# hellojialee/Improved-Body-Parts

Measured on NVIDIA H100. Metric: grouping images/sec @128x128 heatmaps, 30 persons/img, higher is better.
Workload: dtype f32 body-part maps, f32 keypoint maps; f64 coordinates/scores

## Files before the change

### improved_body_parts_b200/csrc/common.cuh

```cuda
#pragma once

#include <cuda_runtime.h>
#include <stdint.h>

#include <algorithm>

namespace spg {

#ifdef SPG_TRACE
constexpr int kTraceCtas = 64, kTraceSlots = 1024;
__device__ unsigned long long g_spg_trace[kTraceCtas * kTraceSlots];
__device__ __forceinline__ void trace_put(int slot, int dep, int mode) {
    if (blockIdx.x < kTraceCtas && (threadIdx.x & 31) == 0) {
        unsigned long long t;
        asm volatile("mov.u64 %0, %%clock64;" : "=l"(t) : "r"(dep) : "memory");
        unsigned long long *w = &g_spg_trace[blockIdx.x * kTraceSlots + slot];
        if (mode == 2) atomicCAS(w, 0ull, t);
        else if (mode == 3) atomicMax(w, t);
        else if (mode == 4) atomicAdd(w, (unsigned long long)(unsigned)dep);
        else *w = mode == 1 ? (unsigned long long)(unsigned)dep : t;
    }
}
#define SPG_TR(slot, dep) ::spg::trace_put((slot), (int)(dep), 0)
#define SPG_TRV(slot, v) ::spg::trace_put((slot), (int)(v), 1)
#define SPG_TR_FIRST(slot, dep) ::spg::trace_put((slot), (int)(dep), 2)
#define SPG_TR_LAST(slot, dep) ::spg::trace_put((slot), (int)(dep), 3)
#define SPG_TR_ADD(slot, v) ::spg::trace_put((slot), (int)(v), 4)
#else
#define SPG_TR(slot, dep) do {} while (0)
#define SPG_TRV(slot, v) do {} while (0)
#define SPG_TR_FIRST(slot, dep) do {} while (0)
#define SPG_TR_LAST(slot, dep) do {} while (0)
#define SPG_TR_ADD(slot, v) do {} while (0)
#endif

constexpr int kMaxParts = 32;
constexpr int kMaxLimbs = 64;
constexpr int kMaxCapPeaks = 128;
constexpr int kMaxCapRows = 128;
constexpr int kMaxRefineRadius = 4;
constexpr int kMaxOutJoints = 32;

constexpr uint32_t kStPeakOverflow = 1u << 0;
constexpr uint32_t kStCandOverflow = 1u << 1;
constexpr uint32_t kStRowOverflow = 1u << 2;
constexpr uint32_t kStSampleIndex = 1u << 3;
constexpr uint32_t kStAssert = 1u << 4;
constexpr uint32_t kStWireOverflow = 1u << 5;

struct Params {
    double thre1, thre2, connect_ration, len_rate, connection_tole, min_mean_score;
    int32_t mid_num, offset_radius, remove_recon, min_parts;
    int32_t crit1_strict, refresh_len_check;
};

struct Workspace {
    int K, L, J, capP, capC, capR, max_batch;
    int16_t limbs[kMaxLimbs * 2];
    int16_t out_from_part[kMaxOutJoints];
    double *peak_x, *peak_y;
    float *peak_score;
    uint32_t *peak_anchor;
    int32_t *peak_count;
    double *cand_prio, *cand_score;
    uint32_t *cand_ij;
    unsigned long long *cand_key;
    int32_t *cand_count;
    int32_t *surv_count;
    uint32_t *conn_ij;
    double *conn_score, *conn_norm;
    int32_t *conn_count;
    double *subset;
    int32_t *n_persons;
    double *people_xy;
    double *people_score;
    uint32_t *status;
    unsigned char *wire;
    long long wire_first;
    int wire_rows;
};

__device__ __forceinline__ uint32_t smem_u32(const void *p) { return (uint32_t)__cvta_generic_to_shared(p); }

__device__ __forceinline__ void mbar_init(uint64_t *bar, uint32_t count) {
    asm volatile("mbarrier.init.shared::cta.b64 [%0], %1;" ::"r"(smem_u32(bar)), "r"(count) : "memory");
}
__device__ __forceinline__ void fence_mbar_init() { asm volatile("fence.mbarrier_init.release.cluster;" ::: "memory"); }
__device__ __forceinline__ void fence_proxy_async() { asm volatile("fence.proxy.async.shared::cta;" ::: "memory"); }
__device__ __forceinline__ void mbar_expect_tx(uint64_t *bar, uint32_t bytes) {
    asm volatile("mbarrier.arrive.expect_tx.shared::cta.b64 _, [%0], %1;" ::"r"(smem_u32(bar)), "r"(bytes) : "memory");
}
__device__ __forceinline__ void bulk_g2s(void *dst_smem, const void *src_gmem, uint32_t bytes, uint64_t *bar) {
    asm volatile("cp.async.bulk.shared::cluster.global.mbarrier::complete_tx::bytes [%0], [%1], %2, [%3];" ::"r"(
                     smem_u32(dst_smem)),
                 "l"(src_gmem), "r"(bytes), "r"(smem_u32(bar))
                 : "memory");
}
__device__ __forceinline__ void mbar_arrive(uint64_t *bar) {
    asm volatile("mbarrier.arrive.shared::cta.b64 _, [%0];" ::"r"(smem_u32(bar)) : "memory");
}
__device__ __forceinline__ bool mbar_try_wait(uint64_t *bar, uint32_t parity) {
    uint32_t ok;
    asm volatile(
        "{\n"
        " .reg .pred p;\n"
        " mbarrier.try_wait.parity.shared::cta.b64 p, [%1], %2;\n"
        " selp.u32 %0, 1, 0, p;\n"
        "}\n"
        : "=r"(ok)
        : "r"(smem_u32(bar)), "r"(parity)
        : "memory");
    return ok != 0;
}
__device__ __forceinline__ void mbar_wait(uint64_t *bar, uint32_t parity) {
    while (!mbar_try_wait(bar, parity)) {
    }
}
__device__ __forceinline__ void mbar_wait_sleep(uint64_t *bar, uint32_t parity, uint32_t hint_ns = 20000u) {
    uint32_t ok = 0;
    while (!ok) {
        asm volatile(
            "{\n"
            " .reg .pred p;\n"
            " mbarrier.try_wait.parity.shared::cta.b64 p, [%1], %2, %3;\n"
            " selp.u32 %0, 1, 0, p;\n"
            "}\n"
            : "=r"(ok)
            : "r"(smem_u32(bar)), "r"(parity), "r"(hint_ns)
            : "memory");
    }
}

template <typename T>
__device__ __forceinline__ T pairwise_sum(const T *a, int n) {
    if (n < 8) {
        T res = (T)0;
        for (int i = 0; i < n; i++) res = res + a[i];
        return res;
    }
    T r[8];
#pragma unroll
    for (int k = 0; k < 8; k++) r[k] = a[k];
    int i = 8;
    for (; i < n - (n % 8); i += 8) {
#pragma unroll
        for (int k = 0; k < 8; k++) r[k] = r[k] + a[i + k];
    }
    T res = ((r[0] + r[1]) + (r[2] + r[3])) + ((r[4] + r[5]) + (r[6] + r[7]));
    for (; i < n; i++) res = res + a[i];
    return res;
}

}
```

### improved_body_parts_b200/csrc/limb_score_persist.cuh

```cuda
#pragma once

#include "limb_score.cuh"

namespace spg {

constexpr int kPersistThreads = 1024;
constexpr int kPersistSlots = 3;
constexpr int kMetaSlots = 5;
constexpr int kWorkerWarps = kPersistThreads / 32 - 1;
constexpr int kPersistMaxCapP = 64;
constexpr int kScreenTailBypass = 4;
constexpr int kPersistListCap = 1024;

constexpr int kTrItemWords = 16, kTrItems = 64;
#define SPG_TR_ITEM(kind, j, f, dep) do { if ((j) < kTrItems) kind(kTrItemWords * (j) + (f), dep); } while (0)

struct PersistHdr {
    int nA, nB, npairs, n, k, special;
    uint32_t magic;
    int pad;
};

struct alignas(16) PeakSlot {
    double ax[kPersistMaxCapP], ay[kPersistMaxCapP], bx[kPersistMaxCapP], by[kPersistMaxCapP];
    float as[kPersistMaxCapP], bs[kPersistMaxCapP];
    float2 fa[kPersistMaxCapP], fb[kPersistMaxCapP];
    unsigned char ain[kPersistMaxCapP], bin[kPersistMaxCapP];
};

struct alignas(16) MetaSlot {
    PeakSlot peaks;
    uint16_t list[kPersistListCap];
    PersistHdr hdr;
    int nsurv, ncand, bnext;
    uint32_t flags;
};

constexpr size_t kPersistPlaneOffset = (screen_tables_bytes() + kMetaSlots * sizeof(MetaSlot) + 127) & ~(size_t)127;
inline size_t persist_smem_bytes(size_t plane_bytes, int ) {
    const size_t plane = (plane_bytes + 127) & ~(size_t)127;
    return kPersistPlaneOffset + kPersistSlots * plane + 128;
}

constexpr uint32_t kScreenBias = 0x4B400000u >> 6;

struct ScreenCtx {
    const PeakSlot *ps;
    uint32_t base;
    const ScreenTab *tab;
    const float *ts;
    int W, mid_num, nB;
    uint32_t magic;
    float thre2;
};

__device__ __forceinline__ void screen_pair(const ScreenCtx &c, int pc, bool valid, int &fails, int &qn, int &maxfail) {
    const int i = c.nB > 1 ? (int)__umulhi((uint32_t)pc, c.magic) : pc;
    const int jj = pc - i * c.nB;
    const float2 fa = c.ps->fa[i], fb = c.ps->fb[jj];
    const float dx64 = fb.x - fa.x, dy64 = fb.y - fa.y;
    const float n2 = (dx64 * dx64 + dy64 * dy64) * (1.0f / 4096.0f);
    float rs;
    asm("rsqrt.approx.ftz.f32 %0, %1;" : "=f"(rs) : "f"(n2));
    const float qf = n2 * rs + 1.0f;
    const float r = rintf(qf);
    const bool longp = qf >= (float)c.mid_num + 0.51f;
    int m = longp ? c.mid_num : min((int)r, c.mid_num);
    if (!longp && !(fabsf(qf - r) < 0.49f)) m = 0;
    if (!(n2 > 1e-6f) || !valid || fminf(fa.x, fb.x) < 0.0f) m = 0;
    m = max(m, 0);
    const ScreenTab tb = c.tab[m];
    qn = tb.qn;
    maxfail = tb.maxfail;
    const float sx64 = dx64 * tb.inv, sy64 = dy64 * tb.inv;
    const float ax64o = fa.x + 33.0f, ay64o = fa.y + 33.0f;
    const float *ts = c.ts + m * kScreenSamples;
    const int qmax = __reduce_max_sync(0xffffffffu, qn);
    const uint32_t base = c.base;
    fails = 0;
    auto sample = [&](int q2) {
        const float tf = ts[q2];
        const uint32_t xb = __float_as_uint(__fadd_rn(__fmaf_rn(tf, sx64, ax64o), 12582912.0f));
        const uint32_t yb = __float_as_uint(__fadd_rn(__fmaf_rn(tf, sy64, ay64o), 12582912.0f));
        float v;
        asm("ld.shared.f32 %0, [%1];" : "=f"(v) : "r"(base + 4u * ((yb >> 6) * (uint32_t)c.W + (xb >> 6))));
        fails += (int)(min(xb & 63u, yb & 63u) > 2u) & (int)!(v > c.thre2);
    };
    if (qmax == kScreenSamples) {
#pragma unroll
        for (int q2 = 0; q2 < kScreenSamples; q2++) sample(q2);
    } else {
#pragma unroll
        for (int q2 = 0; q2 < kScreenSamples; q2++) {
            if (q2 >= qmax) break;
            sample(q2);
        }
    }
    maxfail += qmax - qn;
}

template <typename TA>
__global__ void __launch_bounds__(kPersistThreads, 1) limb_score_persist_kernel(ScoreArgs a, int n_items) {
    extern __shared__ __align__(128) unsigned char smem_raw[];
    __shared__ uint64_t bar_full[kPersistSlots], bar_screened[kMetaSlots], bar_mfree[kMetaSlots];
    __shared__ uint32_t s_bias_bytes;

    using T = float;
    const Workspace &ws = a.ws;
    const int tid = threadIdx.x, lane = tid & 31, warp = tid >> 5;
    const int H = a.H, W = a.W, capP = ws.capP, L = ws.L;
    const size_t plane_bytes = (size_t)H * W * sizeof(T);
    const size_t plane_stride = (plane_bytes + 127) & ~(size_t)127;
    double *s_rcp = reinterpret_cast<double *>(smem_raw);
    ScreenTab *s_tab = reinterpret_cast<ScreenTab *>(s_rcp + (kScreenMaxMid + 1));
    float *s_ts = reinterpret_cast<float *>(s_tab + (kScreenMaxMid + 1));
    MetaSlot *s_meta = reinterpret_cast<MetaSlot *>(smem_raw + screen_tables_bytes());
    unsigned char *s_planes = smem_raw + kPersistPlaneOffset;
    const int nE = min(max(a.exact_warps, 1), kWorkerWarps - 1), nS = kWorkerWarps - nE;

    if (tid == 0) {
        for (int s = 0; s < kPersistSlots; s++) {
            mbar_init(&bar_full[s], 2);
        }
        for (int e = 0; e < kMetaSlots; e++) {
            mbar_init(&bar_screened[e], nS);
            mbar_init(&bar_mfree[e], nE);
            s_meta[e].nsurv = 0; s_meta[e].ncand = 0; s_meta[e].bnext = 0; s_meta[e].flags = 0;
        }
        s_bias_bytes = 4u * kScreenBias * (uint32_t)(W + 1);
        fence_mbar_init();
    }
    if (tid >= 32 && tid < 32 + kScreenMaxMid + 1) build_screen_row(a, tid - 32, s_rcp, s_tab, s_ts, true);
    __syncthreads();

    const int G = gridDim.x;
    const int nj = ((int)blockIdx.x < n_items) ? (n_items - 1 - (int)blockIdx.x) / G + 1 : 0;
    const bool screen = a.screen && a.mid_num <= kScreenMaxMid && H <= kScreenMaxDim && W <= kScreenMaxDim;
    const T thre2 = sizeof(TA) == 8 ? f32_not_above(a.thre2) : (T)a.thre2;
    const TA thre2_exact = (TA)a.thre2;
    auto plane_of = [&](int n_local, int k) {
        return reinterpret_cast<const T *>(a.paf) + (int64_t)n_local * a.img_stride + (int64_t)k * a.chan_stride;
    };

    if (warp == 0) {
        constexpr int kMaxE = kPersistMaxCapP / 32;
        double r_xa[kMaxE], r_ya[kMaxE], r_xb[kMaxE], r_yb[kMaxE];
        float r_sa[kMaxE], r_sb[kMaxE];
        int r_cntA = 0, r_cntB = 0;
        auto fetch = [&](int j) {
            const int item = (int)blockIdx.x + j * G;
            const int n_local = item / L, k = item - n_local * L;
            const int n = a.image_base + n_local;
            const int pa = ws.limbs[2 * k], pb = ws.limbs[2 * k + 1];
            r_cntA = ws.peak_count[(size_t)n * ws.K + pa];
            r_cntB = ws.peak_count[(size_t)n * ws.K + pb];
            const size_t baseA = ((size_t)n * ws.K + pa) * capP, baseB = ((size_t)n * ws.K + pb) * capP;
#pragma unroll
            for (int u = 0; u < kMaxE; u++) {
                const int e = lane + 32 * u;
                if (e < capP) {
                    r_xa[u] = ws.peak_x[baseA + e]; r_ya[u] = ws.peak_y[baseA + e];
                    r_xb[u] = ws.peak_x[baseB + e]; r_yb[u] = ws.peak_y[baseB + e];
                    r_sa[u] = ws.peak_score[baseA + e]; r_sb[u] = ws.peak_score[baseB + e];
                }
            }
        };
        auto close_item = [&](int jp) {
            if (lane == 0) {
                MetaSlot &ms = s_meta[jp % kMetaSlots];
                SPG_TR_ITEM(SPG_TR, jp, 8, ms.nsurv);
                SPG_TR_ITEM(SPG_TRV, jp, 9, ms.nsurv);
                SPG_TR_ITEM(SPG_TRV, jp, 10, ms.ncand);
                publish_limb(ws, ms.hdr.n, (size_t)ms.hdr.n * L + ms.hdr.k, ms.hdr.special ? -1 : ms.ncand, ms.nsurv, ms.flags);
                ms.nsurv = 0; ms.ncand = 0; ms.bnext = 0; ms.flags = 0;
            }
            __syncwarp();
        };
        if (nj > 0) fetch(0);
        for (int j = 0; j < nj; j++) {
            const int s = j % kPersistSlots, e = j % kMetaSlots;
            SPG_TR_ITEM(SPG_TR, j, 0, j);
            if (j >= kPersistSlots) {
                const int jp = j - kPersistSlots;
                mbar_wait_sleep(&bar_screened[jp % kMetaSlots], (jp / kMetaSlots) & 1);
            }
            const int item = (int)blockIdx.x + j * G;
            const int n_local = item / L, k = item - n_local * L;
            const int n = a.image_base + n_local;
            if (lane == 0) {
                const unsigned char *gplane = reinterpret_cast<const unsigned char *>(plane_of(n_local, k));
                unsigned char *dst = s_planes + s * plane_stride;
                mbar_expect_tx(&bar_full[s], (uint32_t)plane_bytes);
                for (size_t off = 0; off < plane_bytes; off += kBulkChunkBytes) {
                    const uint32_t bytes = (uint32_t)min((size_t)kBulkChunkBytes, plane_bytes - off);
                    bulk_g2s(dst + off, gplane + off, bytes, &bar_full[s]);
                }
            }
            SPG_TR_ITEM(SPG_TR, j, 1, j);
            if (j >= kMetaSlots) {
                SPG_TR_ITEM(SPG_TR, j, 2, j);
                mbar_wait_sleep(&bar_mfree[e], ((j / kMetaSlots) - 1) & 1);
                SPG_TR_ITEM(SPG_TR, j, 3, j);
                close_item(j - kMetaSlots);
            }
            MetaSlot &ms = s_meta[e];
            PeakSlot &ps = ms.peaks;
#pragma unroll
            for (int u = 0; u < kMaxE; u++) {
                const int q = lane + 32 * u;
                if (q < capP) {
                    const double xa = r_xa[u], ya = r_ya[u], xb = r_xb[u], yb = r_yb[u];
                    ps.ax[q] = xa; ps.ay[q] = ya; ps.bx[q] = xb; ps.by[q] = yb;
                    ps.as[q] = r_sa[u]; ps.bs[q] = r_sb[u];
                    const bool ain = inside_map(xa, ya, H, W), bin = inside_map(xb, yb, H, W);
                    ps.fa[q] = ain ? make_float2((float)(xa * 64.0), (float)(ya * 64.0)) : make_float2(-1.0f, 0.0f);
                    ps.fb[q] = bin ? make_float2((float)(xb * 64.0), (float)(yb * 64.0)) : make_float2(-1.0f, 0.0f);
                    ps.ain[q] = ain;
                    ps.bin[q] = bin;
                }
            }
            const int nA = min(r_cntA, capP), nB = min(r_cntB, capP);
            const bool special = nA == 0 || nB == 0;
            if (lane == 0) {
                PersistHdr h;
                h.nA = nA; h.nB = nB; h.npairs = special ? 0 : nA * nB; h.n = n; h.k = k; h.special = special;
                h.magic = nB > 1 ? 0xffffffffu / (uint32_t)nB + 1u : 0u;
                h.pad = 0;
                ms.hdr = h;
            }
            __syncwarp();
            SPG_TR_ITEM(SPG_TR, j, 4, j);
            if (lane == 0) mbar_arrive(&bar_full[s]);
            if (j + 1 < nj) fetch(j + 1);
        }
        for (int jp = max(0, nj - kMetaSlots); jp < nj; jp++) {
            mbar_wait_sleep(&bar_mfree[jp % kMetaSlots], (jp / kMetaSlots) & 1);
            close_item(jp);
        }
    } else {
        auto exact_one = [&](MetaSlot &ms, const T *plane, int p) {
            const PersistHdr &h = ms.hdr;
            const PeakSlot &ps = ms.peaks;
            const int nB = h.nB;
            const int i = nB > 1 ? (int)__umulhi((uint32_t)p, h.magic) : p;
            const int jj = p - i * nB;
            PairGeom g{ps.ax, ps.ay, ps.bx, ps.by, ps.as, ps.bs, s_rcp};
            double score, prio;
            bool bad = false;
            const bool ok = score_pair_exact<T, 10, TA>(plane, H, W, a, g, i, jj, ps.ain[i] && ps.bin[jj], thre2_exact, score, prio, bad);
            if (bad) atomicOr(&ms.flags, kStSampleIndex);
            if (ok) {
                const size_t out_base = ((size_t)h.n * L + h.k) * ws.capC;
                const int pos = atomicAdd(&ms.ncand, 1);
                if (pos < ws.capC) store_candidate<TA>(ws, out_base, pos, i, jj, score, prio);
            }
        };

        if (warp <= nS) {
            int c0 = warp - 1;
            for (int j = 0; j < nj; j++) {
                const int s = j % kPersistSlots, e = j % kMetaSlots;
                mbar_wait_sleep(&bar_full[s], (j / kPersistSlots) & 1);
                SPG_TR_ITEM(SPG_TR_FIRST, j, 5, j);
                MetaSlot &ms = s_meta[e];
                const int npairs = ms.hdr.npairs;
                if (c0 * 32 < npairs) {
                    const T *plane = reinterpret_cast<const T *>(s_planes + s * plane_stride);
                    const ScreenCtx sc{&ms.peaks, smem_u32(plane) - *(volatile uint32_t *)&s_bias_bytes, s_tab, s_ts, W, a.mid_num,
                                       ms.hdr.nB, ms.hdr.magic, thre2};
                    for (int c = c0; c * 32 < npairs; c += nS) {
                        const int p = c * 32 + lane;
                        bool keep = p < npairs;
                        if (screen && npairs - c * 32 > kScreenTailBypass) {
                            int fails, qn, maxfail;
                            screen_pair(sc, min(p, npairs - 1), keep, fails, qn, maxfail);
                            if (qn > 0) keep = fails <= maxfail;
                        }
                        const uint32_t km = __ballot_sync(0xffffffffu, keep);
                        if (km) {
                            int at = 0;
                            if (lane == 0) at = atomicAdd(&ms.nsurv, __popc(km));
                            at = __shfl_sync(0xffffffffu, at, 0);
                            if (keep) {
                                const int at_me = at + __popc(km & ((1u << lane) - 1u));
                                if (at_me < kPersistListCap) ms.list[at_me] = (uint16_t)p;
                                else exact_one(ms, plane, p);
                            }
                        }
                    }
                }
                __syncwarp();
                SPG_TR_ITEM(SPG_TR_FIRST, j, 6, j);
                SPG_TR_ITEM(SPG_TR_LAST, j, 7, j);
                if (lane == 0) mbar_arrive(&bar_screened[e]);
                if (++c0 == nS) c0 = 0;
            }
        } else {
            for (int j = 0; j < nj; j++) {
                const int e = j % kMetaSlots;
                mbar_wait_sleep(&bar_screened[e], (j / kMetaSlots) & 1);
                MetaSlot &ms = s_meta[e];
                const int ns = min(ms.nsurv, kPersistListCap);
                if (ns > 0) {
                    const T *gplane = plane_of(ms.hdr.n - a.image_base, ms.hdr.k);
                    for (;;) {
                        if (*(volatile int *)&ms.bnext * 32 >= ns) break;
                        int c = 0;
                        if (lane == 0) c = atomicAdd(&ms.bnext, 1);
                        c = __shfl_sync(0xffffffffu, c, 0);
                        if (c * 32 >= ns) break;
                        const int t = c * 32 + lane;
                        if (t < ns) exact_one(ms, gplane, ms.list[t]);
                        __syncwarp();
                    }
                }
                __syncwarp();
                SPG_TR_ITEM(SPG_TR_LAST, j, 11, j);
                if (lane == 0) mbar_arrive(&bar_mfree[e]);
            }
        }
    }
}

}
```

### improved_body_parts_b200/csrc/spgroup.cu

```cuda
#include "../../include/spgroup.h"

#include <cuda_runtime.h>

#include <algorithm>
#include <cmath>
#include <cstdarg>
#include <cstdio>
#include <cstdlib>
#include <cstring>
#include <new>
#include <string>
#include <vector>

#include "assemble.cuh"
#include "common.cuh"
#include "limb_match.cuh"
#include "limb_score.cuh"
#include "limb_score_persist.cuh"
#include "match_assemble.cuh"
#include "nms_peaks.cuh"
#include "nms_peaks_persist.cuh"
#include "nms_peaks_banded.cuh"
#include "postnet.cuh"
#include "prenet.cuh"

using namespace spg;

static_assert(sizeof(spg_params) == sizeof(spg::Params), "spg_params layout");

static thread_local std::string g_create_error;

enum : int { kStageNms, kStageScore, kStageMatch, kStageAssemble, kStagePostnet, kStagePrenet, kStageCount };

struct Scratch {
    void *p = nullptr;
    size_t bytes = 0;
};

struct spg_handle {
    spg_config cfg{};
    int device = 0;
    int sm_count = 0;
    size_t smem_optin = 0;
    Workspace ws{};
    std::vector<void *> allocs;
    Scratch in_heat, in_paf;
    unsigned int *done_counter = nullptr;
    unsigned long long *armed_flag = nullptr;
    unsigned long long armed_value = 0;
    Scratch heat_acc;
    Scratch pre_grid;
    cudaStream_t streams[2] = {nullptr, nullptr};
    int64_t launches = 0;
    const char *stage_kernel[kStageCount] = {"", "", "", "", "", ""};
    int persist = 1;
    int screen = 1;
    int exact_warps = 14;
    int ma_warps = kMAMatchWarps;
    int fuse_ma = 1;
    int cand_dtype = SPG_F32;
    int stage = 0;
    std::string err;
};

namespace {

int fail(spg_handle *h, int code, const char *fmt, ...) {
    char buf[512];
    va_list ap;
    va_start(ap, fmt);
    vsnprintf(buf, sizeof buf, fmt, ap);
    va_end(ap);
    if (h) h->err = buf; else g_create_error = buf;
    return code;
}

#define SPG_CUDA(h, call)                                                                              \
    do {                                                                                               \
        cudaError_t e_ = (call);                                                                       \
        if (e_ != cudaSuccess) return fail((h), SPG_E_CUDA, "%s failed: %s", #call, cudaGetErrorString(e_)); \
    } while (0)

template <typename T>
int dalloc(spg_handle *h, T **p, size_t count) {
    void *q = nullptr;
    SPG_CUDA(h, cudaMalloc(&q, std::max<size_t>(count, 1) * sizeof(T)));
    h->allocs.push_back(q);
    *p = static_cast<T *>(q);
    return SPG_OK;
}

struct DeviceGuard {
    int prev = -1;
    explicit DeviceGuard(int dev) {
        cudaGetDevice(&prev);
        if (prev != dev) cudaSetDevice(dev);
    }
    ~DeviceGuard() {
        int cur = -1;
        cudaGetDevice(&cur);
        if (prev >= 0 && cur != prev) cudaSetDevice(prev);
    }
};

int grow(spg_handle *h, Scratch &s, size_t bytes) {
    if (s.bytes >= bytes) return SPG_OK;
    if (s.p) cudaFree(s.p);
    s.p = nullptr;
    s.bytes = 0;
    SPG_CUDA(h, cudaMalloc(&s.p, bytes));
    s.bytes = bytes;
    return SPG_OK;
}

template <typename... P, typename... A>
int launch(spg_handle *h, int stage, const char *name, void (*kern)(P...), dim3 grid, int block, size_t smem, cudaStream_t st,
           const A &...args) {
    if (smem > 0) SPG_CUDA(h, cudaFuncSetAttribute(kern, cudaFuncAttributeMaxDynamicSharedMemorySize, (int)smem));
    kern<<<grid, block, smem, st>>>(args...);
    h->stage_kernel[stage] = name;
    h->launches++;
    SPG_CUDA(h, cudaGetLastError());
    return SPG_OK;
}

int check_batch(spg_handle *h, int n) {
    if (n < 0 || n > h->cfg.max_batch) return fail(h, SPG_E_INVALID, "n_images %d outside [0, max_batch=%d]", n, h->cfg.max_batch);
    return SPG_OK;
}

int check_dims(spg_handle *h, int n, int H, int W) {
    int rc;
    if ((rc = check_batch(h, n))) return rc;
    if (H < 2 || W < 2 || H > h->cfg.max_h || W > h->cfg.max_w || H > 32767 || W > 32767)
        return fail(h, SPG_E_INVALID, "map %dx%d outside [2, %dx%d]", H, W, h->cfg.max_h, h->cfg.max_w);
    return SPG_OK;
}

int check_params(spg_handle *h, const spg_params *p) {
    if (!p) return fail(h, SPG_E_INVALID, "params is NULL");
    if (p->offset_radius < 0 || p->offset_radius > kMaxRefineRadius)
        return fail(h, SPG_E_INVALID, "offset_radius %d outside [0, %d]", p->offset_radius, kMaxRefineRadius);
    if (p->mid_num < 1) return fail(h, SPG_E_INVALID, "mid_num must be >= 1");
    return SPG_OK;
}

int check_dtype(spg_handle *h, int dtype) {
    if (dtype != SPG_F32 && dtype != SPG_F64 && dtype != SPG_F32_AS_F64)
        return fail(h, SPG_E_INVALID, "paf_dtype must be SPG_F32, SPG_F64 or SPG_F32_AS_F64");
    return SPG_OK;
}

struct ScoreKernels {
    size_t esz;
    void (*item[2])(ScoreArgs);
    const char *item_name[2];
    void (*ragged[2])(ScoreArgs, ScoreRagged);
    const char *ragged_name[2];
    void (*persist)(ScoreArgs, int);
    const char *persist_name;
};

static_assert(SPG_F32 == 0 && SPG_F64 == 1 && SPG_F32_AS_F64 == 2, "kScoreKernels is indexed by the dtype");
const ScoreKernels kScoreKernels[3] = {
    {4, {limb_score_kernel<float, false>, limb_score_kernel<float, true>},
     {"limb_score_kernel<float,false>", "limb_score_kernel<float,true>"},
     {limb_score_ragged_kernel<float, false>, limb_score_ragged_kernel<float, true>},
     {"limb_score_ragged_kernel<float,false>", "limb_score_ragged_kernel<float,true>"},
     limb_score_persist_kernel<float>, "limb_score_persist_kernel<float>"},
    {8, {limb_score_kernel<double, false>, limb_score_kernel<double, true>},
     {"limb_score_kernel<double,false>", "limb_score_kernel<double,true>"},
     {limb_score_ragged_kernel<double, false>, limb_score_ragged_kernel<double, true>},
     {"limb_score_ragged_kernel<double,false>", "limb_score_ragged_kernel<double,true>"},
     nullptr, ""},
    {4, {limb_score_kernel<float, false, double>, limb_score_kernel<float, true, double>},
     {"limb_score_kernel<float,false,double>", "limb_score_kernel<float,true,double>"},
     {limb_score_ragged_kernel<float, false, double>, limb_score_ragged_kernel<float, true, double>},
     {"limb_score_ragged_kernel<float,false,double>", "limb_score_ragged_kernel<float,true,double>"},
     limb_score_persist_kernel<double>, "limb_score_persist_kernel<double>"},
};

void (*const kNmsPersistKernels[])(NmsArgs, int) = {nms_peaks_persist_kernel<0>, nms_peaks_persist_kernel<1>, nms_peaks_persist_kernel<2>,
                                                    nms_peaks_persist_kernel<3>, nms_peaks_persist_kernel<4>};
static_assert(kMaxRefineRadius == 4, "one nms_peaks_persist_kernel instantiation per radius");

struct NmsPlan {
    enum { kPersist, kBanded, kBands } kind;
    int band_rows, use_bulk;
    size_t smem;
    NmsBanding bg;
};

int plan_nms(spg_handle *h, const float *heat, int64_t img_stride, int64_t chan_stride, int H, int W, bool persistent, int image,
             NmsPlan *pl) {
    const int capP = h->ws.capP;
    *pl = NmsPlan{};
    pl->use_bulk = (W % 4 == 0) && (img_stride % 4 == 0) && (chan_stride % 4 == 0) && ((reinterpret_cast<uintptr_t>(heat) & 15) == 0);
    const bool persist = persistent && h->persist && pl->use_bulk;
    if (persist && nms_persist_smem_bytes(H, W, capP) <= h->smem_optin && (size_t)H * W / 4 < 65536 &&
        (size_t)H * W * sizeof(float) < (1u << 20) &&
        ((size_t)H * W / 4 + kNmsPScanners - 1) / kNmsPScanners <= (size_t)32 * kNmsPMaxIter) {
        pl->kind = NmsPlan::kPersist;
        pl->smem = nms_persist_smem_bytes(H, W, capP);
        return SPG_OK;
    }
    if (persist) pl->bg = nms_banding(H, W, capP, h->smem_optin - 1024);
    if (pl->bg.slots >= kNmsBTeams) {
        pl->kind = NmsPlan::kBanded;
        pl->band_rows = pl->bg.band_rows;
        pl->smem = pl->bg.smem;
        return SPG_OK;
    }
    pl->kind = NmsPlan::kBands;
    pl->band_rows = std::max(4, std::min(H, 4096 / W));
    pl->smem = nms_smem_bytes(pl->band_rows, H, W, capP);
    if (pl->smem <= h->smem_optin) return SPG_OK;
    if (image < 0)
        return fail(h, SPG_E_INVALID, "map width %d needs %zu B of shared memory per band (limit %zu)", W, pl->smem, h->smem_optin);
    return fail(h, SPG_E_INVALID, "image %d: map width %d needs %zu B of shared memory per band (limit %zu)", image, W, pl->smem,
                h->smem_optin);
}

struct ScorePlan {
    enum { kSampled, kStaged, kPersist } kind;
    size_t smem;
};

ScorePlan plan_score(const spg_handle *h, const ScoreKernels &k, const void *paf, int64_t img_stride, int64_t chan_stride, int H,
                     int W, bool persistent) {
    const int capP = h->ws.capP;
    const size_t plane_bytes = (size_t)H * W * k.esz;
    const bool aligned = (plane_bytes % 16 == 0) && ((img_stride * k.esz) % 16 == 0) && ((chan_stride * k.esz) % 16 == 0) &&
                         ((reinterpret_cast<uintptr_t>(paf) & 15) == 0) && plane_bytes < (1u << 20);
    if (persistent && h->persist && k.persist && aligned && capP <= kPersistMaxCapP && persist_smem_bytes(plane_bytes, capP) <= h->smem_optin)
        return {ScorePlan::kPersist, persist_smem_bytes(plane_bytes, capP)};
    const size_t staged = score_smem_bytes(plane_bytes, capP);
    if (aligned && staged <= h->smem_optin) return {ScorePlan::kStaged, staged};
    return {ScorePlan::kSampled, score_smem_bytes(0, capP)};
}

NmsArgs nms_args(const spg_handle *h, const spg_params *p) {
    NmsArgs a{};
    a.radius = p->offset_radius;
    a.thr = (float)p->thre1;
    a.ws = h->ws;
    return a;
}

ScoreArgs score_args(const spg_handle *h, const spg_params *p) {
    ScoreArgs a{};
    a.mid_num = p->mid_num;
    a.thre2 = p->thre2;
    a.connect_ration = p->connect_ration;
    a.screen = h->screen;
    a.crit1_strict = p->crit1_strict != 0;
    a.exact_warps = h->exact_warps;
    a.ws = h->ws;
    return a;
}

AssembleArgs assemble_args(const spg_handle *h, int base, int n, const spg_params *p) {
    AssembleArgs a{};
    a.n_images = n;
    a.image_base = base;
    a.len_rate = p->len_rate;
    a.connection_tole = p->connection_tole;
    a.min_mean_score = p->min_mean_score;
    a.remove_recon = p->remove_recon;
    a.min_parts = p->min_parts;
    a.refresh_len_check = p->refresh_len_check != 0;
    a.wire_flag = h->armed_flag; a.wire_flag_value = h->armed_value; a.done_counter = h->done_counter;
    a.ws = h->ws;
    a.ws.wire_first += base;
    return a;
}

int launch_nms(spg_handle *h, const float *heat, int64_t img_stride, int64_t chan_stride, int base, int n, int H, int W,
               const spg_params *p, cudaStream_t st) {
    if (n == 0) return SPG_OK;
    NmsPlan pl;
    int rc;
    if ((rc = plan_nms(h, heat, img_stride, chan_stride, H, W, true, -1, &pl))) return rc;
    NmsArgs a = nms_args(h, p);
    a.heat = heat;
    a.img_stride = img_stride;
    a.chan_stride = chan_stride;
    a.H = H;
    a.W = W;
    a.band_rows = pl.band_rows;
    a.use_bulk = pl.use_bulk;
    a.image_base = base;
    const int items = n * h->ws.K;
    switch (pl.kind) {
        case NmsPlan::kPersist:
            return launch(h, kStageNms, "nms_peaks_persist_kernel", kNmsPersistKernels[a.radius], std::min(items, h->sm_count),
                          kNmsPThreads, pl.smem, st, a, items);
        case NmsPlan::kBanded:
            return launch(h, kStageNms, "nms_peaks_banded_kernel", nms_peaks_banded_kernel, std::min(items, h->sm_count), kNmsPThreads,
                          pl.smem, st, a, items, pl.bg.slots, pl.bg.n_bands);
        default:
            return launch(h, kStageNms, "nms_peaks_kernel", nms_peaks_kernel, items, kNmsThreads, pl.smem, st, a);
    }
}

int launch_score(spg_handle *h, const void *paf, int dtype, int64_t img_stride, int64_t chan_stride, int base, int n, int H,
                 int W, double extent, const spg_params *p, cudaStream_t st) {
    if (n == 0) return SPG_OK;
    const ScoreKernels &k = kScoreKernels[dtype];
    ScoreArgs a = score_args(h, p);
    a.paf = paf;
    a.img_stride = img_stride;
    a.chan_stride = chan_stride;
    a.H = H;
    a.W = W;
    a.image_base = base;
    a.image_extent = extent;
    h->cand_dtype = dtype;
    const ScorePlan pl = plan_score(h, k, paf, img_stride, chan_stride, H, W, true);
    const int grid = n * h->ws.L;
    if (pl.kind == ScorePlan::kPersist)
        return launch(h, kStageScore, k.persist_name, k.persist, std::min(grid, h->sm_count), kPersistThreads, pl.smem, st, a, grid);
    return launch(h, kStageScore, k.item_name[pl.kind], k.item[pl.kind], grid, kScoreThreads, pl.smem, st, a);
}

template <typename Args, typename Ragged, typename Image>
int launch_ragged(spg_handle *h, int stage, const char *name, void (*kern)(Args, Ragged), int per_image, int block, size_t smem,
                  cudaStream_t st, const Args &a, const std::vector<Image> &imgs) {
    constexpr size_t cap = sizeof(Ragged::img) / sizeof(Image);
    for (size_t i0 = 0; i0 < imgs.size(); i0 += cap) {
        const size_t cnt = std::min(cap, imgs.size() - i0);
        Ragged r{};
        std::copy(imgs.begin() + i0, imgs.begin() + i0 + cnt, r.img);
        int rc;
        if ((rc = launch(h, stage, name, kern, (int)cnt * per_image, block, smem, st, a, r))) return rc;
    }
    return SPG_OK;
}

int launch_match(spg_handle *h, int base, int n, cudaStream_t st) {
    if (n == 0) return SPG_OK;
    MatchArgs a{};
    a.n_images = n;
    a.image_base = base;
    a.keys_valid = h->cand_dtype == SPG_F32;
    a.ws = h->ws;
    const int warps = n * h->ws.L;
    const int blocks = (warps * 32 + kMatchThreads - 1) / kMatchThreads;
    return launch(h, kStageMatch, "limb_match_kernel", limb_match_kernel, blocks, kMatchThreads, 0, st, a);
}

int launch_assemble(spg_handle *h, int base, int n, const spg_params *p, cudaStream_t st) {
    if (n == 0) return SPG_OK;
    AssembleArgs a = assemble_args(h, base, n, p);
    h->armed_flag = nullptr;
    a.use_bulk = ((size_t)h->ws.L * h->ws.capP * sizeof(uint32_t)) % 16 == 0;
    const size_t smem = assemble_smem_bytes(h->ws.K, h->ws.capP, h->ws.capR) + assemble_conn_bytes(h->ws.L, h->ws.capP);
    if (smem > h->smem_optin) return fail(h, SPG_E_INVALID, "capacities need %zu B of shared memory in assemble (limit %zu)", smem, h->smem_optin);
    return launch(h, kStageAssemble, "assemble_kernel", assemble_kernel, n, kAssembleThreads, smem, st, a);
}

int launch_match_assemble(spg_handle *h, int base, int n, const spg_params *p, cudaStream_t st) {
    if (n == 0) return SPG_OK;
    AssembleArgs a = assemble_args(h, base, n, p);
    a.use_bulk = ((size_t)h->ws.K * h->ws.capP * sizeof(float)) % 16 == 0;
    const size_t smem = match_assemble_smem_bytes(h->ws.K, h->ws.L, h->ws.capP, h->ws.capR, h->ma_warps);
    if (smem > h->smem_optin) {
        int rc;
        if ((rc = launch_match(h, base, n, st))) return rc;
        return launch_assemble(h, base, n, p, st);
    }
    h->armed_flag = nullptr;
    h->stage_kernel[kStageAssemble] = "";
    return launch(h, kStageMatch, "match_assemble_kernel", match_assemble_kernel, n, 32 * (1 + h->ma_warps), smem, st, a,
                  h->cand_dtype == SPG_F32);
}

int launch_people(spg_handle *h, int base, int n, const spg_params *p, cudaStream_t st) {
    if (h->fuse_ma) return launch_match_assemble(h, base, n, p, st);
    int rc;
    if ((rc = launch_match(h, base, n, st))) return rc;
    return launch_assemble(h, base, n, p, st);
}

int run_all(spg_handle *h, const float *heat, int64_t his, int64_t hcs, const void *paf, int dtype, int64_t pis, int64_t pcs,
            int base, int n, int H, int W, double extent, const spg_params *p, cudaStream_t st) {
    int rc;
    SPG_CUDA(h, cudaMemsetAsync(h->ws.status + base, 0, sizeof(uint32_t) * (size_t)n, st));
    if ((rc = launch_nms(h, heat, his, hcs, base, n, H, W, p, st))) return rc;
    if ((rc = launch_score(h, paf, dtype, pis, pcs, base, n, H, W, extent, p, st))) return rc;
    return launch_people(h, base, n, p, st);
}

__global__ void wire_signal_kernel(unsigned long long *word, unsigned long long value) {
    __threadfence_system();
    asm volatile("st.release.sys.global.u64 [%0], %1;" ::"l"(word), "l"(value) : "memory");
}

struct WireWords {
    unsigned long long *p[32];
    int n;
};
__global__ void wire_signal_many_kernel(WireWords w, unsigned long long value) {
    __threadfence_system();
    if ((int)threadIdx.x < w.n) asm volatile("st.release.sys.global.u64 [%0], %1;" ::"l"(w.p[threadIdx.x]), "l"(value) : "memory");
}

__global__ void wire_wait_kernel(const unsigned long long *word, unsigned long long value) {
    unsigned long long v;
    do {
        asm volatile("ld.acquire.sys.global.u64 %0, [%1];" : "=l"(v) : "l"(word) : "memory");
        if (v < value) __nanosleep(500);
    } while (v < value);
}

}

extern "C" {

#ifdef SPG_TRACE
int spg_trace_read(unsigned long long *out, size_t n_words, int clear) {
    const size_t n = std::min(n_words, (size_t)spg::kTraceCtas * spg::kTraceSlots);
    if (cudaMemcpyFromSymbol(out, spg::g_spg_trace, n * sizeof(unsigned long long)) != cudaSuccess) return -1;
    if (clear) {
        void *p = nullptr;
        if (cudaGetSymbolAddress(&p, spg::g_spg_trace) != cudaSuccess) return -1;
        if (cudaMemset(p, 0, sizeof(spg::g_spg_trace)) != cudaSuccess) return -1;
    }
    return 0;
}
#endif

int spg_abi_version(void) { return SPG_ABI_VERSION; }

const char *spg_last_error(const spg_handle *h) { return h ? h->err.c_str() : g_create_error.c_str(); }

int spg_create(const spg_config *cfg, spg_handle **out) {
    if (!cfg || !out) return fail(nullptr, SPG_E_INVALID, "cfg/out is NULL");
    *out = nullptr;
    if (cfg->abi_version != SPG_ABI_VERSION) return fail(nullptr, SPG_E_INVALID, "ABI version %d != %d", cfg->abi_version, SPG_ABI_VERSION);
    if (cfg->n_parts < 1 || cfg->n_parts > kMaxParts || cfg->n_limbs < 1 || cfg->n_limbs > kMaxLimbs || !cfg->limbs)
        return fail(nullptr, SPG_E_INVALID, "n_parts in [1,%d], n_limbs in [1,%d], limbs non-NULL required", kMaxParts, kMaxLimbs);
    if (cfg->n_out_joints < 0 || cfg->n_out_joints > kMaxOutJoints || (cfg->n_out_joints && !cfg->out_from_part))
        return fail(nullptr, SPG_E_INVALID, "n_out_joints in [0,%d]", kMaxOutJoints);
    if (cfg->max_peaks_per_part < 1 || cfg->max_peaks_per_part > kMaxCapPeaks)
        return fail(nullptr, SPG_E_INVALID, "max_peaks_per_part in [1,%d]", kMaxCapPeaks);
    if (cfg->max_person_rows < 1 || cfg->max_person_rows > kMaxCapRows)
        return fail(nullptr, SPG_E_INVALID, "max_person_rows in [1,%d]", kMaxCapRows);
    if (cfg->max_cands_per_limb < 1 || cfg->max_batch < 1 || cfg->max_h < 2 || cfg->max_w < 2)
        return fail(nullptr, SPG_E_INVALID, "max_cands_per_limb, max_batch >= 1 and max_h, max_w >= 2 required");
    for (int k = 0; k < cfg->n_limbs * 2; k++)
        if (cfg->limbs[k] < 0 || cfg->limbs[k] >= cfg->n_parts) return fail(nullptr, SPG_E_INVALID, "limb table entry %d out of range", k);
    for (int g = 0; g < cfg->n_out_joints; g++)
        if (cfg->out_from_part[g] < 0 || cfg->out_from_part[g] >= cfg->n_parts) return fail(nullptr, SPG_E_INVALID, "out_from_part[%d] out of range", g);

    int ndev = 0;
    if (cudaGetDeviceCount(&ndev) != cudaSuccess || ndev == 0) return fail(nullptr, SPG_E_NO_DEVICE, "no CUDA device (this library has no CPU path)");
    if (cfg->device < 0 || cfg->device >= ndev) return fail(nullptr, SPG_E_INVALID, "device %d outside [0,%d)", cfg->device, ndev);
    cudaDeviceProp prop{};
    if (cudaGetDeviceProperties(&prop, cfg->device) != cudaSuccess) return fail(nullptr, SPG_E_CUDA, "cudaGetDeviceProperties failed");
    if (prop.major != 9 || prop.minor != 0) return fail(nullptr, SPG_E_NO_DEVICE, "device %d is sm_%d%d; this library is built for sm_90a only", cfg->device, prop.major, prop.minor);

    spg_handle *h = new (std::nothrow) spg_handle();
    if (!h) return fail(nullptr, SPG_E_INVALID, "out of host memory");
    h->cfg = *cfg;
    h->cfg.limbs = nullptr;
    h->cfg.out_from_part = nullptr;
    h->device = cfg->device;
    h->sm_count = prop.multiProcessorCount;
    h->smem_optin = prop.sharedMemPerBlockOptin;
    if (const char *e = getenv("SPG_NO_SCREEN")) h->screen = !(e[0] == '1');
    if (const char *e = getenv("SPG_PERSIST")) h->persist = !(e[0] == '0');
    if (const char *e = getenv("SPG_MA_WARPS")) h->ma_warps = std::max(1, std::min(15, atoi(e)));
    if (const char *e = getenv("SPG_FUSE_MA")) h->fuse_ma = !(e[0] == '0');
    if (const char *e = getenv("SPG_EXACT_WARPS")) h->exact_warps = std::max(1, std::min(30, atoi(e)));
    DeviceGuard guard(h->device);

    const size_t N = cfg->max_batch, K = cfg->n_parts, L = cfg->n_limbs, J = cfg->n_out_joints;
    const size_t cP = cfg->max_peaks_per_part, cC = cfg->max_cands_per_limb, cR = cfg->max_person_rows;
    Workspace &ws = h->ws;
    ws.K = (int)K; ws.L = (int)L; ws.J = (int)J; ws.capP = (int)cP; ws.capC = (int)cC; ws.capR = (int)cR; ws.max_batch = (int)N;
    int rc = SPG_OK;
    auto A = [&](int r) { if (rc == SPG_OK) rc = r; };
    A(dalloc(h, &ws.peak_x, N * K * cP));
    A(dalloc(h, &ws.peak_y, N * K * cP));
    A(dalloc(h, &ws.peak_score, N * K * cP));
    A(dalloc(h, &ws.peak_anchor, N * K * cP));
    A(dalloc(h, &ws.peak_count, N * K));
    A(dalloc(h, &ws.cand_prio, N * L * cC));
    A(dalloc(h, &ws.cand_score, N * L * cC));
    A(dalloc(h, &ws.cand_ij, N * L * cC));
    A(dalloc(h, &ws.cand_key, N * L * cC));
    A(dalloc(h, &ws.cand_count, N * L));
    A(dalloc(h, &ws.surv_count, N * L));
    A(dalloc(h, &ws.conn_ij, N * L * cP));
    A(dalloc(h, &ws.conn_score, N * L * cP));
    A(dalloc(h, &ws.conn_norm, N * L * cP));
    A(dalloc(h, &ws.conn_count, N * L));
    A(dalloc(h, &ws.subset, N * cR * (K + 2) * 2));
    A(dalloc(h, &ws.n_persons, N));
    A(dalloc(h, &ws.people_xy, N * cR * std::max<size_t>(J, 1) * 2));
    A(dalloc(h, &ws.people_score, N * cR));
    A(dalloc(h, &ws.status, N));
    for (size_t i = 0; i < L * 2; i++) ws.limbs[i] = (int16_t)cfg->limbs[i];
    for (size_t g = 0; g < J; g++) ws.out_from_part[g] = (int16_t)cfg->out_from_part[g];
    if (rc == SPG_OK && cudaMemset(ws.status, 0, sizeof(uint32_t) * N) != cudaSuccess) rc = SPG_E_CUDA;
    if (rc == SPG_OK && cudaMemset(ws.peak_count, 0, sizeof(int32_t) * N * K) != cudaSuccess) rc = SPG_E_CUDA;
    for (int s = 0; s < 2 && rc == SPG_OK; s++)
        if (cudaStreamCreateWithFlags(&h->streams[s], cudaStreamNonBlocking) != cudaSuccess) rc = SPG_E_CUDA;
    if (rc != SPG_OK) {
        g_create_error = h->err.empty() ? "device allocation failed" : h->err;
        spg_destroy(h);
        return rc;
    }
    *out = h;
    return SPG_OK;
}

void spg_destroy(spg_handle *h) {
    if (!h) return;
    DeviceGuard guard(h->device);
    cudaDeviceSynchronize();
    for (void *p : h->allocs) cudaFree(p);
    for (Scratch *s : {&h->in_heat, &h->in_paf, &h->heat_acc, &h->pre_grid})
        if (s->p) cudaFree(s->p);
    if (h->done_counter) cudaFree(h->done_counter);
    for (auto &s : h->streams)
        if (s) cudaStreamDestroy(s);
    delete h;
}

int spg_get_device_view(const spg_handle *h, spg_device_view *v) {
    if (!h || !v) return SPG_E_INVALID;
    const Workspace &ws = h->ws;
    v->max_batch = ws.max_batch; v->n_parts = ws.K; v->n_limbs = ws.L; v->n_out_joints = ws.J;
    v->cap_peaks = ws.capP; v->cap_cands = ws.capC; v->cap_rows = ws.capR;
    v->peak_x = ws.peak_x; v->peak_y = ws.peak_y; v->peak_score = ws.peak_score; v->peak_anchor = ws.peak_anchor;
    v->peak_count = ws.peak_count;
    v->conn_ij = ws.conn_ij; v->conn_score = ws.conn_score; v->conn_norm = ws.conn_norm; v->conn_count = ws.conn_count;
    v->cand_count = ws.cand_count;
    v->surv_count = ws.surv_count;
    v->subset = ws.subset; v->n_persons = ws.n_persons; v->people_xy = ws.people_xy; v->people_score = ws.people_score;
    v->status = ws.status;
    return SPG_OK;
}

int64_t spg_wire_record_bytes(const spg_handle *h) {
    if (!h) return 0;
    const int rows = h->ws.wire_rows > 0 ? h->ws.wire_rows : h->ws.capR;
    return 8 + (int64_t)rows * (2 * h->ws.J + 2) * (int64_t)sizeof(double);
}

int spg_set_wire_output(spg_handle *h, void *wire_dev, int64_t first_record, int32_t wire_rows) {
    if (!h) return SPG_E_INVALID;
    if (!wire_dev) {
        h->ws.wire = nullptr;
        h->ws.wire_first = 0;
        return SPG_OK;
    }
    if (wire_rows < 1 || wire_rows > h->ws.capR) return fail(h, SPG_E_INVALID, "wire_rows %d outside [1, max_person_rows=%d]", wire_rows, h->ws.capR);
    if (first_record < 0) return fail(h, SPG_E_INVALID, "first_record is negative");
    if ((reinterpret_cast<uintptr_t>(wire_dev) & 7) != 0) return fail(h, SPG_E_INVALID, "wire buffer must be 8-byte aligned");
    if ((size_t)wire_rows * (2 * h->ws.J + 2) * sizeof(double) > assemble_conn_bytes(h->ws.L, h->ws.capP))
        return fail(h, SPG_E_INVALID, "wire_rows %d do not fit the assemble kernel's staging area", wire_rows);
    h->ws.wire = static_cast<unsigned char *>(wire_dev);
    h->ws.wire_first = first_record;
    h->ws.wire_rows = wire_rows;
    return SPG_OK;
}

int spg_arm_wire_signal(spg_handle *h, uint64_t *word_dev, uint64_t value) {
    if (!h) return SPG_E_INVALID;
    if (!word_dev) {
        h->armed_flag = nullptr;
        return SPG_OK;
    }
    if (!h->ws.wire) return fail(h, SPG_E_STATE, "spg_arm_wire_signal needs a wire output (spg_set_wire_output) first");
    if (!h->done_counter) {
        DeviceGuard guard(h->device);
        SPG_CUDA(h, cudaMalloc(&h->done_counter, sizeof(unsigned int)));
        SPG_CUDA(h, cudaMemset(h->done_counter, 0, sizeof(unsigned int)));
    }
    h->armed_flag = reinterpret_cast<unsigned long long *>(word_dev);
    h->armed_value = value;
    return SPG_OK;
}

int spg_wire_create(int32_t device, uint64_t bytes, void **dev_ptr, unsigned char ipc_handle[64]) {
    if (!dev_ptr || !ipc_handle || bytes == 0) return SPG_E_INVALID;
    static_assert(sizeof(cudaIpcMemHandle_t) == 64, "IPC handle size");
    DeviceGuard guard(device);
    void *p = nullptr;
    if (cudaMalloc(&p, bytes) != cudaSuccess) return fail(nullptr, SPG_E_CUDA, "cudaMalloc of %llu wire bytes failed", (unsigned long long)bytes);
    cudaIpcMemHandle_t hd;
    if (cudaMemset(p, 0, bytes) != cudaSuccess || cudaDeviceSynchronize() != cudaSuccess || cudaIpcGetMemHandle(&hd, p) != cudaSuccess) {
        const char *why = cudaGetErrorString(cudaGetLastError());
        cudaFree(p);
        return fail(nullptr, SPG_E_CUDA, "exporting the wire buffer failed: %s", why);
    }
    memcpy(ipc_handle, &hd, 64);
    *dev_ptr = p;
    return SPG_OK;
}

int spg_wire_open(int32_t device, const unsigned char ipc_handle[64], void **peer_ptr) {
    if (!peer_ptr || !ipc_handle) return SPG_E_INVALID;
    DeviceGuard guard(device);
    cudaIpcMemHandle_t hd;
    memcpy(&hd, ipc_handle, 64);
    void *p = nullptr;
    const cudaError_t e = cudaIpcOpenMemHandle(&p, hd, cudaIpcMemLazyEnablePeerAccess);
    if (e != cudaSuccess) {
        cudaGetLastError();
        return fail(nullptr, SPG_E_CUDA, "cudaIpcOpenMemHandle failed: %s (no peer access between the two GPUs?)", cudaGetErrorString(e));
    }
    *peer_ptr = p;
    return SPG_OK;
}

int spg_wire_close(void *peer_ptr) { return (!peer_ptr || cudaIpcCloseMemHandle(peer_ptr) == cudaSuccess) ? SPG_OK : SPG_E_CUDA; }

int spg_wire_destroy(int32_t device, void *dev_ptr) {
    if (!dev_ptr) return SPG_OK;
    DeviceGuard guard(device);
    cudaDeviceSynchronize();
    return cudaFree(dev_ptr) == cudaSuccess ? SPG_OK : SPG_E_CUDA;
}

int spg_wire_signal(int32_t device, uint64_t *word_dev, uint64_t value, void *stream) {
    if (!word_dev) return SPG_E_INVALID;
    DeviceGuard guard(device);
    wire_signal_kernel<<<1, 1, 0, static_cast<cudaStream_t>(stream)>>>(reinterpret_cast<unsigned long long *>(word_dev), value);
    return cudaGetLastError() == cudaSuccess ? SPG_OK : fail(nullptr, SPG_E_CUDA, "wire_signal launch failed");
}

int spg_wire_signal_many(int32_t device, uint64_t *const *words_dev, int32_t n_words, uint64_t value, void *stream) {
    if (!words_dev || n_words < 1 || n_words > 32) return SPG_E_INVALID;
    DeviceGuard guard(device);
    WireWords w{};
    w.n = n_words;
    for (int i = 0; i < n_words; i++) {
        if (!words_dev[i]) return SPG_E_INVALID;
        w.p[i] = reinterpret_cast<unsigned long long *>(words_dev[i]);
    }
    wire_signal_many_kernel<<<1, 32, 0, static_cast<cudaStream_t>(stream)>>>(w, value);
    return cudaGetLastError() == cudaSuccess ? SPG_OK : fail(nullptr, SPG_E_CUDA, "wire_signal_many launch failed");
}

int spg_wire_wait(int32_t device, const uint64_t *word_dev, uint64_t value, void *stream) {
    if (!word_dev) return SPG_E_INVALID;
    DeviceGuard guard(device);
    typedef int (*wait_fn_t)(cudaStream_t, unsigned long long, unsigned long long, unsigned int);
    static wait_fn_t wait_fn = nullptr;
    static bool looked = false;
    if (!looked) {
        void *fn = nullptr;
        cudaDriverEntryPointQueryResult q;
        if (cudaGetDriverEntryPoint("cuStreamWaitValue64", &fn, cudaEnableDefault, &q) == cudaSuccess && q == cudaDriverEntryPointSuccess)
            wait_fn = reinterpret_cast<wait_fn_t>(fn);
        cudaGetLastError();
// ... 550 lines not shown
```

Baseline: 564,600.

## Replace static strided item assignment with atomic work queue in persistent score kernel

The persistent limb-scoring kernel now pulls work items dynamically from a global atomic counter instead of each CTA taking a fixed stride of items. A sentinel item (npairs = -1) propagates termination through the producer, screener and exact-scoring warps, and the last CTA to finish resets the queue for the next launch. This targets load imbalance between CTAs whose items have uneven peak counts. In exchange it adds an atomic per item, a grid-wide completion counter, and a per-stream queue, and makes the item-to-CTA mapping nondeterministic. CTA span tracing is also added, but only under SPG_TRACE.

```diff
diff --git a/improved_body_parts_b200/csrc/common.cuh b/improved_body_parts_b200/csrc/common.cuh
--- a/improved_body_parts_b200/csrc/common.cuh
+++ b/improved_body_parts_b200/csrc/common.cuh
@@ -26,12 +26,26 @@
 #define SPG_TR_FIRST(slot, dep) ::spg::trace_put((slot), (int)(dep), 2)
 #define SPG_TR_LAST(slot, dep) ::spg::trace_put((slot), (int)(dep), 3)
 #define SPG_TR_ADD(slot, v) ::spg::trace_put((slot), (int)(v), 4)
+constexpr int kTraceSpanCtas = 1024;
+__device__ unsigned long long g_spg_cta_span[kTraceSpanCtas * 2];
+__device__ __forceinline__ void trace_cta(int exit) {
+    if (blockIdx.x < kTraceSpanCtas && (threadIdx.x & 31) == 0 && (exit || threadIdx.x == 0)) {
+        unsigned long long t;
+        asm volatile("mov.u64 %0, %%globaltimer;" : "=l"(t) :: "memory");
+        if (exit) atomicMax(&g_spg_cta_span[2 * blockIdx.x + 1], t);
+        else g_spg_cta_span[2 * blockIdx.x] = t;
+    }
+}
+#define SPG_TR_CTA_START() ::spg::trace_cta(0)
+#define SPG_TR_CTA_EXIT() ::spg::trace_cta(1)
 #else
 #define SPG_TR(slot, dep) do {} while (0)
 #define SPG_TRV(slot, v) do {} while (0)
 #define SPG_TR_FIRST(slot, dep) do {} while (0)
 #define SPG_TR_LAST(slot, dep) do {} while (0)
 #define SPG_TR_ADD(slot, v) do {} while (0)
+#define SPG_TR_CTA_START() do {} while (0)
+#define SPG_TR_CTA_EXIT() do {} while (0)
 #endif
 
 constexpr int kMaxParts = 32;
diff --git a/improved_body_parts_b200/csrc/limb_score_persist.cuh b/improved_body_parts_b200/csrc/limb_score_persist.cuh
--- a/improved_body_parts_b200/csrc/limb_score_persist.cuh
+++ b/improved_body_parts_b200/csrc/limb_score_persist.cuh
@@ -100,10 +100,11 @@
 }
 
 template <typename TA>
-__global__ void __launch_bounds__(kPersistThreads, 1) limb_score_persist_kernel(ScoreArgs a, int n_items) {
+__global__ void __launch_bounds__(kPersistThreads, 1) limb_score_persist_kernel(ScoreArgs a, int n_items, unsigned int *queue) {
     extern __shared__ __align__(128) unsigned char smem_raw[];
     __shared__ uint64_t bar_full[kPersistSlots], bar_screened[kMetaSlots], bar_mfree[kMetaSlots];
     __shared__ uint32_t s_bias_bytes;
+    SPG_TR_CTA_START();
 
     using T = float;
     const Workspace &ws = a.ws;
@@ -133,8 +134,6 @@
     if (tid >= 32 && tid < 32 + kScreenMaxMid + 1) build_screen_row(a, tid - 32, s_rcp, s_tab, s_ts, true);
     __syncthreads();
 
-    const int G = gridDim.x;
-    const int nj = ((int)blockIdx.x < n_items) ? (n_items - 1 - (int)blockIdx.x) / G + 1 : 0;
     const bool screen = a.screen && a.mid_num <= kScreenMaxMid && H <= kScreenMaxDim && W <= kScreenMaxDim;
     const T thre2 = sizeof(TA) == 8 ? f32_not_above(a.thre2) : (T)a.thre2;
     const TA thre2_exact = (TA)a.thre2;
@@ -146,9 +145,12 @@
         constexpr int kMaxE = kPersistMaxCapP / 32;
         double r_xa[kMaxE], r_ya[kMaxE], r_xb[kMaxE], r_yb[kMaxE];
         float r_sa[kMaxE], r_sb[kMaxE];
-        int r_cntA = 0, r_cntB = 0;
-        auto fetch = [&](int j) {
-            const int item = (int)blockIdx.x + j * G;
+        int r_cntA = 0, r_cntB = 0, r_item = 0;
+        auto fetch = [&]() {
+            int t = 0;
+            if (lane == 0) t = (int)atomicAdd(queue, 1u);
+            r_item = __shfl_sync(0xffffffffu, t, 0);
+            const int item = min(r_item, n_items - 1);
             const int n_local = item / L, k = item - n_local * L;
             const int n = a.image_base + n_local;
             const int pa = ws.limbs[2 * k], pb = ws.limbs[2 * k + 1];
@@ -176,22 +178,24 @@
             }
             __syncwarp();
         };
-        if (nj > 0) fetch(0);
-        for (int j = 0; j < nj; j++) {
+        fetch();
+        int j = 0;
+        for (;; j++) {
             const int s = j % kPersistSlots, e = j % kMetaSlots;
             SPG_TR_ITEM(SPG_TR, j, 0, j);
             if (j >= kPersistSlots) {
                 const int jp = j - kPersistSlots;
                 mbar_wait_sleep(&bar_screened[jp % kMetaSlots], (jp / kMetaSlots) & 1);
             }
-            const int item = (int)blockIdx.x + j * G;
-            const int n_local = item / L, k = item - n_local * L;
+            const bool live = r_item < n_items;
+            const int n_local = r_item / L, k = r_item - n_local * L;
             const int n = a.image_base + n_local;
             if (lane == 0) {
                 const unsigned char *gplane = reinterpret_cast<const unsigned char *>(plane_of(n_local, k));
                 unsigned char *dst = s_planes + s * plane_stride;
-                mbar_expect_tx(&bar_full[s], (uint32_t)plane_bytes);
-                for (size_t off = 0; off < plane_bytes; off += kBulkChunkBytes) {
+                const size_t bytes_in = live ? plane_bytes : 0;
+                mbar_expect_tx(&bar_full[s], (uint32_t)bytes_in);
+                for (size_t off = 0; off < bytes_in; off += kBulkChunkBytes) {
                     const uint32_t bytes = (uint32_t)min((size_t)kBulkChunkBytes, plane_bytes - off);
                     bulk_g2s(dst + off, gplane + off, bytes, &bar_full[s]);
                 }
@@ -223,7 +227,7 @@
             const bool special = nA == 0 || nB == 0;
             if (lane == 0) {
                 PersistHdr h;
-                h.nA = nA; h.nB = nB; h.npairs = special ? 0 : nA * nB; h.n = n; h.k = k; h.special = special;
+                h.nA = nA; h.nB = nB; h.npairs = !live ? -1 : special ? 0 : nA * nB; h.n = n; h.k = k; h.special = special;
                 h.magic = nB > 1 ? 0xffffffffu / (uint32_t)nB + 1u : 0u;
                 h.pad = 0;
                 ms.hdr = h;
@@ -231,11 +235,20 @@
             __syncwarp();
             SPG_TR_ITEM(SPG_TR, j, 4, j);
             if (lane == 0) mbar_arrive(&bar_full[s]);
-            if (j + 1 < nj) fetch(j + 1);
-        }
-        for (int jp = max(0, nj - kMetaSlots); jp < nj; jp++) {
+            if (!live) break;
+            fetch();
+        }
+        for (int jp = max(0, j - kMetaSlots + 1); jp < j; jp++) {
             mbar_wait_sleep(&bar_mfree[jp % kMetaSlots], (jp / kMetaSlots) & 1);
             close_item(jp);
+        }
+        if (lane == 0) {
+            __threadfence();
+            if (atomicAdd(queue + 1, 1u) == gridDim.x - 1) {
+                __threadfence();
+                *(volatile unsigned int *)queue = 0u;
+                *(volatile unsigned int *)(queue + 1) = 0u;
+            }
         }
     } else {
         auto exact_one = [&](MetaSlot &ms, const T *plane, int p) {
@@ -258,7 +271,7 @@
 
         if (warp <= nS) {
             int c0 = warp - 1;
-            for (int j = 0; j < nj; j++) {
+            for (int j = 0;; j++) {
                 const int s = j % kPersistSlots, e = j % kMetaSlots;
                 mbar_wait_sleep(&bar_full[s], (j / kPersistSlots) & 1);
                 SPG_TR_ITEM(SPG_TR_FIRST, j, 5, j);
@@ -293,13 +306,15 @@
                 SPG_TR_ITEM(SPG_TR_FIRST, j, 6, j);
                 SPG_TR_ITEM(SPG_TR_LAST, j, 7, j);
                 if (lane == 0) mbar_arrive(&bar_screened[e]);
+                if (npairs < 0) break;
                 if (++c0 == nS) c0 = 0;
             }
         } else {
-            for (int j = 0; j < nj; j++) {
+            for (int j = 0;; j++) {
                 const int e = j % kMetaSlots;
                 mbar_wait_sleep(&bar_screened[e], (j / kMetaSlots) & 1);
                 MetaSlot &ms = s_meta[e];
+                if (ms.hdr.npairs < 0) break;
                 const int ns = min(ms.nsurv, kPersistListCap);
                 if (ns > 0) {
                     const T *gplane = plane_of(ms.hdr.n - a.image_base, ms.hdr.k);
@@ -320,6 +335,7 @@
             }
         }
     }
+    SPG_TR_CTA_EXIT();
 }
 
 }
diff --git a/improved_body_parts_b200/csrc/spgroup.cu b/improved_body_parts_b200/csrc/spgroup.cu
--- a/improved_body_parts_b200/csrc/spgroup.cu
+++ b/improved_body_parts_b200/csrc/spgroup.cu
@@ -46,6 +46,7 @@
     std::vector<void *> allocs;
     Scratch in_heat, in_paf;
     unsigned int *done_counter = nullptr;
+    unsigned int *score_queue = nullptr;
     unsigned long long *armed_flag = nullptr;
     unsigned long long armed_value = 0;
     Scratch heat_acc;
@@ -157,7 +158,7 @@
     const char *item_name[2];
     void (*ragged[2])(ScoreArgs, ScoreRagged);
     const char *ragged_name[2];
-    void (*persist)(ScoreArgs, int);
+    void (*persist)(ScoreArgs, int, unsigned int *);
     const char *persist_name;
 };
 
@@ -318,8 +319,11 @@
     h->cand_dtype = dtype;
     const ScorePlan pl = plan_score(h, k, paf, img_stride, chan_stride, H, W, true);
     const int grid = n * h->ws.L;
-    if (pl.kind == ScorePlan::kPersist)
-        return launch(h, kStageScore, k.persist_name, k.persist, std::min(grid, h->sm_count), kPersistThreads, pl.smem, st, a, grid);
+    if (pl.kind == ScorePlan::kPersist) {
+        unsigned int *queue = h->score_queue + (st == h->streams[1] ? 2 : 0);
+        return launch(h, kStageScore, k.persist_name, k.persist, std::min(grid, h->sm_count), kPersistThreads, pl.smem, st, a, grid,
+                      queue);
+    }
     return launch(h, kStageScore, k.item_name[pl.kind], k.item[pl.kind], grid, kScoreThreads, pl.smem, st, a);
 }
 
@@ -425,6 +429,16 @@
         void *p = nullptr;
         if (cudaGetSymbolAddress(&p, spg::g_spg_trace) != cudaSuccess) return -1;
         if (cudaMemset(p, 0, sizeof(spg::g_spg_trace)) != cudaSuccess) return -1;
+    }
+    return 0;
+}
+int spg_trace_read_spans(unsigned long long *out, size_t n_words, int clear) {
+    const size_t n = std::min(n_words, (size_t)2 * spg::kTraceSpanCtas);
+    if (cudaMemcpyFromSymbol(out, spg::g_spg_cta_span, n * sizeof(unsigned long long)) != cudaSuccess) return -1;
+    if (clear) {
+        void *p = nullptr;
+        if (cudaGetSymbolAddress(&p, spg::g_spg_cta_span) != cudaSuccess) return -1;
+        if (cudaMemset(p, 0, sizeof(spg::g_spg_cta_span)) != cudaSuccess) return -1;
     }
     return 0;
 }
@@ -501,10 +515,12 @@
     A(dalloc(h, &ws.people_xy, N * cR * std::max<size_t>(J, 1) * 2));
     A(dalloc(h, &ws.people_score, N * cR));
     A(dalloc(h, &ws.status, N));
+    A(dalloc(h, &h->score_queue, 4));
     for (size_t i = 0; i < L * 2; i++) ws.limbs[i] = (int16_t)cfg->limbs[i];
     for (size_t g = 0; g < J; g++) ws.out_from_part[g] = (int16_t)cfg->out_from_part[g];
     if (rc == SPG_OK && cudaMemset(ws.status, 0, sizeof(uint32_t) * N) != cudaSuccess) rc = SPG_E_CUDA;
     if (rc == SPG_OK && cudaMemset(ws.peak_count, 0, sizeof(int32_t) * N * K) != cudaSuccess) rc = SPG_E_CUDA;
+    if (rc == SPG_OK && cudaMemset(h->score_queue, 0, sizeof(unsigned int) * 4) != cudaSuccess) rc = SPG_E_CUDA;
     for (int s = 0; s < 2 && rc == SPG_OK; s++)
         if (cudaStreamCreateWithFlags(&h->streams[s], cudaStreamNonBlocking) != cudaSuccess) rc = SPG_E_CUDA;
     if (rc != SPG_OK) {
```

Result: faster. 596,000 (median of 6 runs) (+5.6%).
